# olegiy/manuscript-ocr

Hardware: AMD Instinct MI355X
Metric: manuscript pages/sec end-to-end (EAST+TRBA) at 1/2/4/8 MI355X; CER vs CPU ref (higher is better)
Workload: dtype f32 (bf16x3 split operands on the 1x1 / Winograd-domain GEMMs, f32 accumulate)

## Files before the change

### include/msocr.h

```cpp
#ifndef MSOCR_H
#define MSOCR_H
#include <stdint.h>

#ifdef __cplusplus
extern "C" {
#endif

#define MSOCR_F32 0
#define MSOCR_BF16 1

#define MSOCR_OK 0
#define MSOCR_E_ARG (-1)
#define MSOCR_E_LAUNCH (-2)
#define MSOCR_E_NOGPU (-3)

#define MSOCR_CONV_RELU 1u
#define MSOCR_CONV_RESIDUAL 2u
#define MSOCR_CONV_POOL2 4u

typedef struct msocr_conv_desc {
  int32_t dtype;
  int32_t N, H, W, Cin;
  int64_t in_sN, in_sH, in_sW;
  int32_t KH, KW, stride_h, stride_w, pad_h, pad_w;
  int32_t Ho, Wo, Cout;
  int64_t out_ld;
  int64_t res_ld;
  uint32_t flags;
} msocr_conv_desc;

int msocr_conv2d(const msocr_conv_desc* d, const void* in, const void* weight, const float* bias,
                 const void* residual, void* out, void* stream);

#define MSOCR_WINO_2X2 0
#define MSOCR_WINO_4X2 1
#define MSOCR_WINO_4X4 2
#define MSOCR_WINO_4X4_COLTAIL 3
int64_t msocr_winograd_workspace_bytes(const msocr_conv_desc* d, int form);
int msocr_winograd_weights_host(int form, const float* w_khwc_host, int Cout, int Cin, float* u_out_host);
int msocr_conv3x3_winograd(const msocr_conv_desc* d, int form, int split, const void* in, const void* u, const float* bias,
                           const void* residual, void* out, void* workspace, void* stream);
int msocr_winograd_input_transform(const msocr_conv_desc* d, int form, const void* in, void* workspace, void* stream);
int msocr_winograd_gemm(const msocr_conv_desc* d, int form, int split, const void* u, void* workspace, void* stream);
int msocr_winograd_output_transform(const msocr_conv_desc* d, int form, const void* workspace, const float* bias, const void* residual,
                                    void* out, void* stream);

int64_t msocr_winograd_crop_lds_bytes(const msocr_conv_desc* d, int form, int se);
int msocr_winograd_output_chain(const msocr_conv_desc* d, int form, void* workspace, const float* bias, void* stream);
int msocr_winograd_output_se(const msocr_conv_desc* d, int form, const void* workspace, const float* bias, const void* identity,
                             const float* w1, const float* w2, float* gate_ws, void* out, void* stream);

int msocr_split_bf16x3_host(const float* w_host, int64_t n, uint16_t* planes_out_host);
int msocr_split_bf16x3_ktile_host(const float* w_host, int64_t nbatch, int64_t rows, int64_t k, uint16_t* planes_out_host);
int msocr_conv1x1_split(const msocr_conv_desc* d, const void* in, const void* weight_planes, const float* bias,
                        const void* residual, void* out, void* stream);
int msocr_conv2d_split(const msocr_conv_desc* d, const void* in, const void* weight_planes, const float* bias,
                       const void* residual, void* out, void* stream);

int64_t msocr_winograd_fused64_workspace_bytes(const msocr_conv_desc* d);
int msocr_conv3x3_winograd_fused64(const msocr_conv_desc* d, int split, const void* in, const void* u, const float* bias,
                                   const void* residual, void* out, void* workspace, void* stream);
int msocr_winograd_fused64_gemm_output(const msocr_conv_desc* d, int split, const void* u, const void* workspace, const float* bias,
                                       const void* residual, void* out, void* stream);

int msocr_normalize_u8(const uint8_t* src, int N, int H, int W, int pad_t, int pad_l, int Hp, int Wp, int cpad,
                       int mode, int dtype, void* out, void* stream);

int msocr_resize_linear_u8(const uint8_t* src, int N, int sh, int sw, uint8_t* dst, int dh, int dw, void* stream);

int msocr_maxpool2d(const void* in, int N, int H, int W, int C, int64_t in_ld, int k, int s, int p, int dtype,
                    void* out, int Ho, int Wo, int64_t out_ld, void* stream);

int msocr_upsample2x_bilinear(const void* in, int N, int H, int W, int C, int64_t in_ld, int dtype, void* out,
                              int64_t out_ld, void* stream);

int msocr_east_head(const void* h1, int64_t npix, int64_t in_ld, int dtype, const float* w9, const float* b9,
                    float* score_out, float* geo_out, void* stream);

int msocr_east_decode(const float* score, const float* geo, int N, int H, int W, float thresh, float scale,
                      int quant, float* cand_out, int32_t* count_out, int max_cand, void* stream);

int64_t msocr_lanms_workspace_bytes(int N, int max_cand);
int msocr_east_lanms(const float* cand, const int32_t* counts, int N, int max_cand, double iou_thr, float* boxes_out,
                     int32_t* nbox_out, void* workspace, void* stream);

int64_t msocr_east_box_tail_workspace_bytes(int N, int max_cand);
int msocr_east_box_tail(const float* boxes, const int32_t* nbox, int N, int max_cand, double expand_w, double expand_h,
                        double scale_x, double scale_y, int axis_aligned_output, int remove_anomalies, double sigma, int min_count,
                        float* out, int32_t* n_out, void* workspace, void* stream);
int msocr_east_box_tail_host(const float* quads_host, int M, double expand_w, double expand_h, double scale_x, double scale_y,
// ... 260 lines not shown
```

### manuscript_ocr_amd/_native.py

```python
import ctypes
import os

import torch

_HERE = os.path.dirname(os.path.abspath(__file__))
LIB_PATH = os.path.join(_HERE, "libmsocr.so")

F32, BF16 = 0, 1
CONV_RELU, CONV_RESIDUAL, CONV_POOL2 = 1, 2, 4
WINO_2X2, WINO_4X2, WINO_4X4, WINO_4X4_COLTAIL = 0, 1, 2, 3

c_i32, c_i64, c_u32 = ctypes.c_int32, ctypes.c_int64, ctypes.c_uint32
c_f32, c_f64, c_vp = ctypes.c_float, ctypes.c_double, ctypes.c_void_p


class ConvDesc(ctypes.Structure):
    _fields_ = [
        ("dtype", c_i32), ("N", c_i32), ("H", c_i32), ("W", c_i32), ("Cin", c_i32),
        ("in_sN", c_i64), ("in_sH", c_i64), ("in_sW", c_i64),
        ("KH", c_i32), ("KW", c_i32), ("stride_h", c_i32), ("stride_w", c_i32), ("pad_h", c_i32), ("pad_w", c_i32),
        ("Ho", c_i32), ("Wo", c_i32), ("Cout", c_i32),
        ("out_ld", c_i64), ("res_ld", c_i64), ("flags", c_u32),
    ]

# ... 26 lines not shown

ATTN_GREEDY, ATTN_BEAM, ATTN_FORCED = 0, 1, 2


class AttnDesc(ctypes.Structure):
    _fields_ = (
        [(n, c_i32) for n in ("struct_bytes", "mode", "B", "T", "H", "V", "steps", "beam", "sos_id", "eos_id", "blank_id")]
        + [("temperature", c_f32), ("batch_H", c_vp), ("proj_H", c_vp), ("ctx_gates", c_vp),
           ("w", ctypes.POINTER(AttnWeights)), ("ws", ctypes.POINTER(AttnSplitWeights))]
        + [(n, c_vp) for n in ("lp", "tok_in", "logits_out", "ids_out", "workspace", "fin_step_out", "chunk_id", "chunk_size",
                               "chunk_state", "alpha_out")]
        + [("lexicon", ctypes.POINTER(LexiconArrays)), ("node_out", c_vp), ("lm", ctypes.POINTER(CharLMTable)), ("lm_weight", c_f32),
           ("ctx_out", c_vp)])


_SIGS = {
    "msocr_conv2d": (c_i32, [ctypes.POINTER(ConvDesc), c_vp, c_vp, c_vp, c_vp, c_vp, c_vp]),
    "msocr_winograd_workspace_bytes": (c_i64, [ctypes.POINTER(ConvDesc), c_i32]),
    "msocr_winograd_weights_host": (c_i32, [c_i32, c_vp, c_i32, c_i32, c_vp]),
    "msocr_conv3x3_winograd": (c_i32, [ctypes.POINTER(ConvDesc), c_i32, c_i32, c_vp, c_vp, c_vp, c_vp, c_vp, c_vp, c_vp]),
    "msocr_winograd_input_transform": (c_i32, [ctypes.POINTER(ConvDesc), c_i32, c_vp, c_vp, c_vp]),
    "msocr_winograd_gemm": (c_i32, [ctypes.POINTER(ConvDesc), c_i32, c_i32, c_vp, c_vp, c_vp]),
    "msocr_winograd_output_transform": (c_i32, [ctypes.POINTER(ConvDesc), c_i32, c_vp, c_vp, c_vp, c_vp, c_vp]),
    "msocr_winograd_crop_lds_bytes": (c_i64, [ctypes.POINTER(ConvDesc), c_i32, c_i32]),
    "msocr_winograd_output_chain": (c_i32, [ctypes.POINTER(ConvDesc), c_i32, c_vp, c_vp, c_vp]),
    "msocr_winograd_output_se": (c_i32, [ctypes.POINTER(ConvDesc), c_i32, c_vp, c_vp, c_vp, c_vp, c_vp, c_vp, c_vp, c_vp]),
    "msocr_winograd_fused64_workspace_bytes": (c_i64, [ctypes.POINTER(ConvDesc)]),
    "msocr_conv3x3_winograd_fused64": (c_i32, [ctypes.POINTER(ConvDesc), c_i32, c_vp, c_vp, c_vp, c_vp, c_vp, c_vp, c_vp]),
    "msocr_winograd_fused64_gemm_output": (c_i32, [ctypes.POINTER(ConvDesc), c_i32, c_vp, c_vp, c_vp, c_vp, c_vp, c_vp]),
    "msocr_split_bf16x3_host": (c_i32, [c_vp, c_i64, c_vp]),
    "msocr_split_bf16x3_ktile_host": (c_i32, [c_vp, c_i64, c_i64, c_i64, c_vp]),
    "msocr_conv1x1_split": (c_i32, [ctypes.POINTER(ConvDesc), c_vp, c_vp, c_vp, c_vp, c_vp, c_vp]),
    "msocr_conv2d_split": (c_i32, [ctypes.POINTER(ConvDesc), c_vp, c_vp, c_vp, c_vp, c_vp, c_vp]),
    "msocr_normalize_u8": (c_i32, [c_vp, c_i32, c_i32, c_i32, c_i32, c_i32, c_i32, c_i32, c_i32, c_i32, c_i32, c_vp, c_vp]),
    "msocr_resize_linear_u8": (c_i32, [c_vp, c_i32, c_i32, c_i32, c_vp, c_i32, c_i32, c_vp]),
    "msocr_maxpool2d": (c_i32, [c_vp, c_i32, c_i32, c_i32, c_i32, c_i64, c_i32, c_i32, c_i32, c_i32, c_vp, c_i32, c_i32, c_i64, c_vp]),
    "msocr_upsample2x_bilinear": (c_i32, [c_vp, c_i32, c_i32, c_i32, c_i32, c_i64, c_i32, c_vp, c_i64, c_vp]),
    "msocr_east_head": (c_i32, [c_vp, c_i64, c_i64, c_i32, c_vp, c_vp, c_vp, c_vp, c_vp]),
    "msocr_east_decode": (c_i32, [c_vp, c_vp, c_i32, c_i32, c_i32, c_f32, c_f32, c_i32, c_vp, c_vp, c_i32, c_vp]),
    "msocr_lanms_workspace_bytes": (c_i64, [c_i32, c_i32]),
    "msocr_east_lanms": (c_i32, [c_vp, c_vp, c_i32, c_i32, c_f64, c_vp, c_vp, c_vp, c_vp]),
    "msocr_se_residual": (c_i32, [c_vp, c_vp, c_i32, c_i32, c_i32, c_i32, c_vp, c_vp, c_vp, c_vp, c_vp]),
    "msocr_mean_over_h": (c_i32, [c_vp, c_i32, c_i32, c_i32, c_i32, c_i32, c_vp, c_vp]),
    "msocr_bilstm_recurrent": (c_i32, [c_vp, c_vp, c_i32, c_i32, c_i32, c_vp, c_vp]),
    "msocr_bilstm_recurrent_split": (c_i32, [c_vp, c_vp, c_i32, c_i32, c_i32, c_vp, c_vp]),
    "msocr_attn_pack_split_elems": (c_i64, [c_i32]),
    "msocr_attn_pack_split_host": (c_i32, [c_vp, c_i32, c_i32, c_vp]),
    "msocr_attn_beam_workspace_bytes": (c_i64, [c_i32, c_i32, c_i32, c_i32]),
    "msocr_attn_beam_finalize": (c_i32, [c_vp, c_i32, c_i32, c_i32, c_i32, c_vp, c_vp, c_vp, c_vp, c_i32, c_vp, c_vp]),
    "msocr_attn_beam_slots_bytes": (c_i64, [c_i32, c_i32, c_i32]),
    "msocr_attn_decode": (c_i32, [ctypes.POINTER(AttnDesc), c_vp]),
    "msocr_seq_confidence": (c_i32, [c_vp, c_vp, c_vp, c_i32, c_i32, c_i32, c_vp, c_vp]),
    "msocr_attn_beam_alpha_bytes": (c_i64, [c_i32, c_i32, c_i32, c_i32]),
    "msocr_seq_char_details": (c_i32, [c_vp, c_vp, c_vp, c_vp, c_i32, c_i32, c_i32, c_i32, c_vp, c_vp, c_vp, c_vp]),
    "msocr_attn_beam_nbest": (c_i32, [c_vp, c_i32, c_i32, c_i32, c_i32, c_i32, c_i32, c_vp, c_vp, c_vp, c_vp, c_vp, c_vp]),
    "msocr_attn_beam_nbest_host": (c_i32, [c_vp, c_i32, c_i32, c_i32, c_i32, c_i32, c_i32, c_vp, c_vp, c_vp, c_vp, c_vp]),
    "msocr_seq_logp": (c_i32, [c_vp, c_vp, c_vp, c_i32, c_i32, c_i32, c_f32, c_vp, c_vp, c_vp]),
    "msocr_seq_logp_host": (c_i32, [c_vp, c_vp, c_vp, c_i32, c_i32, c_i32, c_f32, c_vp, c_vp]),
    "msocr_lexicon_check_host": (c_i32, [c_vp, c_vp, c_vp, c_vp, c_i32, c_i32, c_i32, c_i32]),
    "msocr_lexicon_nearest_ws_bytes": (c_i64, [c_i32, c_i32, c_i32]),
    "msocr_lexicon_nearest": (c_i32, [c_vp, c_vp, c_i32, c_i32, c_i32, c_i32, c_i32, c_i32, ctypes.POINTER(WordList), c_i32, c_i32,
                                      c_vp, c_vp, c_vp, c_vp]),
    "msocr_lexicon_nearest_host": (c_i32, [c_vp, c_vp, c_i32, c_i32, c_i32, c_i32, c_i32, c_i32, ctypes.POINTER(WordList), c_i32, c_i32,
                                           c_vp, c_vp]),
    "msocr_edit_distance_pairs": (c_i32, [c_vp, c_vp, c_i32, c_vp, c_vp, c_i32, c_i32, c_i32, c_i32, c_i32, c_i32, c_vp, c_vp, c_vp,
                                          c_vp]),
# ... 105 lines not shown
```

### manuscript_ocr_amd/csrc/conv_common.h

```cpp
#ifndef MSOCR_CONV_COMMON_H
#define MSOCR_CONV_COMMON_H
#include <hip/hip_runtime.h>
#include <stdint.h>

#include <type_traits>

#include "internal.h"
#include "msocr.h"
#include "split_mma.h"

typedef uint32_t u32x4 __attribute__((ext_vector_type(4)));
typedef uint32_t u32x2 __attribute__((ext_vector_type(2)));

struct ConvParams {
  const char* in;
  const char* w;
  const float* bias;
  const char* res;
  char* out;
  int N, H, W, Cin;
  long sN, sH, sW;
  int KH, KW, SH, SW, PH, PW;
  int Ho, Wo, Cout;
  long M;
  int ktiles, cin_tiles;
  long Ktot;
  long out_ld, res_ld;
  int relu, has_res;
  int tilesM, tilesN;
  int nbatch;
  long bsA, bsW, bsO;
  long wplane;
  long w_kt_b;
};

__device__ __forceinline__ float bf16_to_f32(uint16_t v) { return __uint_as_float(((uint32_t)v) << 16); }
__device__ __forceinline__ uint16_t f32_to_bf16(float f) {
  __bf16 b = (__bf16)f;
  return *reinterpret_cast<uint16_t*>(&b);
}

template <typename T>
struct Mma;
template <>
struct Mma<float> {
  static __device__ __forceinline__ void run(const u32x4& a, const u32x4& b, f32x16& c) {
#pragma unroll
    for (int j = 0; j < 4; ++j)
      c = __builtin_amdgcn_mfma_f32_32x32x2f32(__uint_as_float(a[j]), __uint_as_float(b[j]), c, 0, 0, 0);
  }
};
template <>
struct Mma<__bf16> {
  static __device__ __forceinline__ void run(const u32x4& a, const u32x4& b, f32x16& c) {
    bf16x8 av = __builtin_bit_cast(bf16x8, a);
    bf16x8 bv = __builtin_bit_cast(bf16x8, b);
    c = __builtin_amdgcn_mfma_f32_32x32x16_bf16(av, bv, c, 0, 0, 0);
  }
};

__attribute__((visibility("hidden"))) bool msocr_internal_split_pp_takes(const ConvParams& p);
__attribute__((visibility("hidden"))) int msocr_internal_split_pp_launch(ConvParams& p, hipStream_t s, bool general);

template <int BKB>
__device__ __forceinline__ int swz(int row) {
  constexpr int CPR = BKB / 16;
// ... 2 lines not shown
}
__device__ __forceinline__ int swz16(int row) { return (4 - ((row >> 2) & 3)) & 3; }
template <typename T, int BM_, int BN_, int BKB_, int WM_, int STAGES_>
struct IgemmTile {
  static constexpr int BM = BM_, BN = BN_, BKB = BKB_, THREADS = 256, PERSISTENT = 0;
  static constexpr int BK = BKB / (int)sizeof(T);
  static constexpr int CPR = BKB / 16;
  static constexpr int RPP = 256 / CPR;
  static constexpr int A_IT = BM / RPP, B_IT = (BN + RPP - 1) / RPP;
  static constexpr int A_BYTES = BM * BKB, B_BYTES = BN * BKB, STAGE = A_BYTES + B_BYTES;
  static constexpr int EPI = (BM / WM_) * 32 * BN * 4;
  static constexpr int LDS = STAGES_ * STAGE > EPI ? STAGES_ * STAGE : EPI;
};
template <int BM_, int BN_>
struct SplitStage {
  static constexpr int BM = BM_, BN = BN_, BK = 32;
  static constexpr int ROWB = BK * 2;
  static constexpr int A_PLANE = BM * ROWB, B_PLANE = BN * ROWB;
  static constexpr int STAGE_B = 3 * (A_PLANE + B_PLANE);
  static constexpr int ACH = BK / 4, ARP = 256 / ACH, A_IT = BM / ARP;
  static constexpr int BCH = BK / 8, BRP = 256 / BCH, B_IT = (BN + BRP - 1) / BRP;
};
template <int BN_>
struct SplitTile : SplitStage<128, BN_> {
  static constexpr int WM = 64, WN = BN_ / 2, THREADS = 256, PERSISTENT = 0;
  static constexpr int EPI = (128 / WM) * 32 * BN_ * 4;
  static constexpr int LDS = SplitStage<128, BN_>::STAGE_B > EPI ? SplitStage<128, BN_>::STAGE_B : EPI;
  static __device__ __forceinline__ int swz(int row) { return ::swz<64>(row); }
};
template <int TM, int TN>
struct SplitPPTile : SplitStage<64 * TM, 64 * TN> {
  static constexpr int THREADS = 512, PERSISTENT = 1;
  static constexpr int BIAS_OFF = 2 * SplitStage<64 * TM, 64 * TN>::STAGE_B;
  static constexpr int LDS = BIAS_OFF + 4 * 64 * TN * 4;
  static __device__ __forceinline__ int swz(int row) { return swz16(row); }
};

static __device__ __attribute__((aligned(16))) uint32_t msocr_zero16[4] = {0u, 0u, 0u, 0u};

template <typename I>
__device__ __forceinline__ void xcd_range(I x, I nblk, I& first, I& count) {
  const I q = nblk >> 3, r = nblk & 7;
  first = x < r ? x * (q + 1) : r * (q + 1) + (x - r) * q;
  count = q + (x < r ? 1 : 0);
}
template <typename I>
__device__ __forceinline__ I xcd_tile(I bid, I nblk) {
  I first, count;
  xcd_range<I>(bid & 7, nblk, first, count);
  return first + (bid >> 3);
}
__device__ __forceinline__ void tile_coords(const ConvParams& p, int t, int& batch, int& tile_m, int& tile_n) {
  const int nblk1 = p.tilesM * p.tilesN;
  batch = t / nblk1;
  t -= batch * nblk1;
  tile_n = t % p.tilesN;
  tile_m = t / p.tilesN;
}

template <bool GEN>
struct ATap { int hi0, wi0; };
template <>
struct ATap<false> {};
__device__ __forceinline__ long a_row_origin(const ConvParams& p, long m, ATap<true>& t) {
  const long hw = (long)p.Ho * p.Wo;
  const int n = (int)(m / hw);
  const int rem = (int)(m - (long)n * hw);
// ... 42 lines not shown
}
__device__ __forceinline__ uint32_t b_plane_offset(int co, int cout, int b_chunk) {
  if (co >= cout) co = cout - 1;
  return (uint32_t)(co * 64 + b_chunk * 16);
}
template <class G>
__device__ __forceinline__ void load_b_planes(const ConvParams& p, const char* g_w, long wplane_b, int kt, int b_row0,
                                              const uint32_t (&b_off)[G::B_IT], u32x4 (&rb)[3][G::B_IT]) {
#pragma unroll
  for (int pl = 0; pl < 3; ++pl) {
    const char* const gb = g_w + pl * wplane_b + (long)kt * p.w_kt_b;
#pragma unroll
    for (int j = 0; j < G::B_IT; ++j)
      if (G::BN % G::BRP == 0 || b_row0 + j * G::BRP < G::BN) rb[pl][j] = *reinterpret_cast<const u32x4*>(gb + b_off[j]);
  }
}
template <class G>
__device__ __forceinline__ void split_store_row(unsigned char* sA, int row, int a_chunk, u32x4 r) {
  float x0 = __uint_as_float(r[0]), x1 = __uint_as_float(r[1]), x2 = __uint_as_float(r[2]), x3 = __uint_as_float(r[3]);
  unsigned char* dst = sA + row * G::ROWB + (((a_chunk >> 1) ^ G::swz(row)) << 4) + ((a_chunk & 1) << 3);
#pragma unroll
  for (int pl = 0; pl < 3; ++pl) {
    u32x2 v;
    v[0] = split_step(x0, x1);
    v[1] = split_step(x2, x3);
    *reinterpret_cast<u32x2*>(dst + pl * G::A_PLANE) = v;
  }
}
template <class G>
__device__ __forceinline__ void store_b_row(unsigned char* sB, int pl, int row, int b_chunk, u32x4 v) {
  *reinterpret_cast<u32x4*>(sB + pl * G::B_PLANE + row * G::ROWB + ((b_chunk ^ G::swz(row)) << 4)) = v;
}

template <typename T, int BM, int BN, int WM, int WN, int MT, bool BIAS16, int NCH = 1, typename AccT, int TMA, int TN>
__device__ __forceinline__ void epilogue_lds(const ConvParams& p, unsigned char* smem, const AccT (&acc)[TMA][TN], int tile_m, int tile_n,
                                             char* g_out, int wm, int wn, int r32, int half) {
  constexpr int ES = sizeof(T), EPC = 16 / ES;
  constexpr int AE = MT == 32 ? 16 : 4;
  const int tid = threadIdx.x;
  constexpr int PR = (BM / WM) * 32;
  float* sc = reinterpret_cast<float*>(smem);
  constexpr int VPR = BN / EPC;
  constexpr int ROWS_PP = 256 / VPR;
  const int vcol = (tid % VPR) * EPC;
  const int vrow0 = tid / VPR;
  const int co = tile_n * BN + vcol;
  float bias[EPC];
  if constexpr (BIAS16) {
    static_assert(EPC == 4, "four f32");
    f32x4 b = {0.f, 0.f, 0.f, 0.f};
    if (p.bias) b = *reinterpret_cast<const f32x4*>(p.bias + co);
    bias[0] = b[0]; bias[1] = b[1]; bias[2] = b[2]; bias[3] = b[3];
  } else {
#pragma unroll
    for (int e = 0; e < EPC; ++e) bias[e] = p.bias ? p.bias[co + e] : 0.f;
  }

  constexpr int TPP = 32 / MT;
  constexpr int NR = PR / ROWS_PP;
  static_assert(PR % ROWS_PP == 0 && NR % NCH == 0, "a pass is whole sweeps of 256 threads, a chunk whole rows");
  static_assert(32 % ROWS_PP == 0 || ROWS_PP == 64, "tile_row must be additive in the sweep index (see row_step)");
  const long m0 = (long)tile_m * BM;
  auto tile_row = [&](int i, int lr) { return (lr >> 5) * WM + i * 32 + (lr & 31); };
  auto lds_write = [&](int i) {
#pragma unroll
    for (int ti = 0; ti < TPP; ++ti)
// ... 147 lines not shown
  p.nbatch = 1;
  return p;
}
static inline int gemm_params(const void* A, const void* B, void* C, long M, int N, int K, int nbatch, int n_mult, int k_mult, ConvParams* out) {
  if (!A || !B || !C || M <= 0 || N <= 0 || N % n_mult || K <= 0 || K % k_mult || nbatch <= 0) return MSOCR_E_ARG;
  if (((uintptr_t)A | (uintptr_t)B | (uintptr_t)C) & 15) return MSOCR_E_ARG;
  if (M > 0x7fffffffL) return MSOCR_E_ARG;
  ConvParams p = {};
  p.in = (const char*)A; p.w = (const char*)B; p.out = (char*)C;
  p.N = 1; p.H = (int)M; p.W = 1; p.Cin = K;
  p.sN = M * (long)K; p.sH = K; p.sW = K;
  p.KH = p.KW = 1; p.SH = p.SW = 1;
  p.Ho = (int)M; p.Wo = 1; p.Cout = N;
  p.M = M; p.Ktot = K;
  p.out_ld = N;
  p.nbatch = nbatch; p.bsA = M * (long)K; p.bsW = (long)N * K; p.bsO = M * (long)N;
  *out = p;
  return MSOCR_OK;
}
template <class G, class Kern>
static int conv_launch(Kern kern, ConvParams& p, hipStream_t s) {
  p.tilesM = (int)((p.M + G::BM - 1) / G::BM);
  p.tilesN = p.Cout / G::BN;
  p.cin_tiles = p.Cin / G::BK;
  p.ktiles = (int)(p.Ktot / G::BK);
  if (msocr_internal_lds_limit(reinterpret_cast<const void*>(kern), G::LDS) != MSOCR_OK) return MSOCR_E_LAUNCH;
  const long nblk = (long)p.tilesM * p.tilesN * p.nbatch;
  if (nblk <= 0 || nblk > 0x7fffffffL) return MSOCR_E_ARG;
  long grid = nblk;
  if (G::PERSISTENT) {
    int n_cu = 0;
    if (msocr_internal_cu_count(&n_cu) != MSOCR_OK) return MSOCR_E_LAUNCH;
    n_cu = n_cu > 8 ? n_cu & ~7 : 8;
    grid = (nblk + 7) & ~7L;
    if (grid > n_cu) grid = n_cu;
  }
  MSOCR_LAUNCH(kern, dim3((unsigned)grid), dim3(G::THREADS), G::LDS, s, p);
  return hipGetLastError() == hipSuccess ? MSOCR_OK : MSOCR_E_LAUNCH;
}

#endif
```

### manuscript_ocr_amd/csrc/conv_split.hip

```cpp
#include <hip/hip_runtime.h>
#include <stdint.h>
#include <stdlib.h>
#include <string.h>

#include "conv_common.h"

namespace {

template <int BN, int WPE, bool GEN>
__global__ __launch_bounds__(256, WPE) void conv_split_kernel(ConvParams p) {
  using G = SplitTile<BN>;
  constexpr int BM = G::BM, WM = G::WM, WN = G::WN, BK = G::BK;
  constexpr int TM = WM / 32, TN = WN / 32;
  constexpr int ROWB = G::ROWB, A_PLANE = G::A_PLANE, B_PLANE = G::B_PLANE, STAGE_B = G::STAGE_B;
  constexpr int ACH = G::ACH, ARP = G::ARP, A_IT = G::A_IT;
  constexpr int BCH = G::BCH, B_IT = G::B_IT;

  extern __shared__ __attribute__((aligned(16))) unsigned char smem[];

  const int tid = threadIdx.x;
  const int lane = tid & 63;
  const int wave = tid >> 6;
  const int wm = wave >> 1, wn = wave & 1;

// ... 172 lines not shown
  return launch_split_any(p, (hipStream_t)stream, false);
}

extern "C" int msocr_conv2d_split(const msocr_conv_desc* d, const void* in, const void* weight_planes, const float* bias,
                                  const void* residual, void* out, void* stream) {
  if (!d || d->dtype != MSOCR_F32) return MSOCR_E_ARG;
  if (conv_desc_check(d, in, weight_planes, residual, out, 4, 32, 64, CONV_STRIDES_ALIGNED) != MSOCR_OK) return MSOCR_E_ARG;
  ConvParams p = conv_params(d, in, weight_planes, bias, residual, out);
  p.wplane = (long)d->Cout * p.Ktot;
  const long img_bytes = (long)d->in_sN * 4;
  if (img_bytes >= (1L << 31)) return MSOCR_E_ARG;
  const int per = (int)(((1L << 31) - 1) / (img_bytes > 0 ? img_bytes : 1));
  if (d->N <= per) return launch_split_any(p, (hipStream_t)stream, true);
  const long out_img = (long)d->Ho * d->Wo * d->out_ld * 4, res_img = (long)d->Ho * d->Wo * d->res_ld * 4;
  for (int n0 = 0; n0 < d->N; n0 += per) {
    ConvParams q = p;
    q.N = d->N - n0 < per ? d->N - n0 : per;
    q.M = (long)q.N * d->Ho * d->Wo;
    q.in = p.in + (long)n0 * img_bytes;
    q.out = p.out + (long)n0 * out_img;
    if (p.has_res) q.res = p.res + (long)n0 * res_img;
    const int rc = launch_split_any(q, (hipStream_t)stream, true);
    if (rc != MSOCR_OK) return rc;
  }
  return MSOCR_OK;
}

int msocr_internal_gemm_split_batched(const float* A, const uint16_t* Bplanes, float* C, long M, int N, int K, int nbatch, hipStream_t s) {
  ConvParams p;
  if (gemm_params(A, Bplanes, C, M, N, K, nbatch, 64, 32, &p) != MSOCR_OK) return MSOCR_E_ARG;
  p.wplane = (long)nbatch * N * K;
  return launch_split_any(p, s, false);
}
```

### manuscript_ocr_amd/csrc/conv_split_pp.hip

```cpp
#include <hip/hip_runtime.h>
#include <stdint.h>

#include <type_traits>

#include "conv_common.h"

namespace {

template <int I>
using ic = std::integral_constant<int, I>;
template <int U, int N, class F>
__device__ __forceinline__ void static_for(F&& f) {
  if constexpr (U < N) {
    f(ic<U>{});
    static_for<U + 1, N>(f);
  }
}

__device__ __forceinline__ void lds_barrier() {
  __builtin_amdgcn_sched_barrier(0);
  asm volatile("s_waitcnt lgkmcnt(0)\n\ts_barrier" ::: "memory");
  __builtin_amdgcn_sched_barrier(0);
}

template <int OFF>
__device__ __forceinline__ void store_f32x4_saddr(const char* sbase, uint32_t voff, f32x4 v) {
  asm volatile("global_store_dwordx4 %0, %1, %2 offset:%3" ::"v"(voff), "v"(v), "s"(sbase), "n"(OFF) : "memory");
}

template <int TM, int TN, bool GEN>
__global__ __launch_bounds__(512, 2) void conv_split_pp_kernel(ConvParams p) {
  using Tile = SplitPPTile<TM, TN>;
  constexpr int BM = Tile::BM, BN = Tile::BN, BK = Tile::BK, ROWB = Tile::ROWB;
  constexpr int A_PLANE = Tile::A_PLANE, B_PLANE = Tile::B_PLANE, STAGE_B = Tile::STAGE_B;
  constexpr int BIAS_OFF = Tile::BIAS_OFF;
  constexpr int RM = 2 * TM, RN = 2 * TN;
  constexpr bool STREAM_B = TN >= TM;
  constexpr int RH = STREAM_B ? RM : RN, RS = STREAM_B ? RN : RM;

  extern __shared__ __attribute__((aligned(16))) unsigned char smem[];

  const int tid = threadIdx.x;
  const int lane = tid & 63;
  const int wave = __builtin_amdgcn_readfirstlane(tid >> 6);

  const int nblk = p.tilesM * p.tilesN * p.nbatch;
  const int xcd = blockIdx.x & 7, slot = blockIdx.x >> 3, per_x = gridDim.x >> 3;
  int x_start, x_cnt;
  xcd_range<int>(xcd, nblk, x_start, x_cnt);
  const int my_tiles = slot < x_cnt ? (x_cnt - slot + per_x - 1) / per_x : 0;
  const int G = my_tiles * p.ktiles;
  if (G == 0) return;

  auto tile_of = [&](int n, int& batch, int& tile_m, int& tile_n) __attribute__((always_inline)) {
    tile_coords(p, x_start + slot + n * per_x, batch, tile_m, tile_n);
  };

  if (wave >= 4) {
    constexpr int D = 2;
    const int ltid = tid & 255;
    constexpr int ACH = Tile::ACH, ARP = Tile::ARP, A_IT = Tile::A_IT;
    constexpr int BCH = Tile::BCH, B_IT = Tile::B_IT;
    const int a_chunk = ltid % ACH, a_row0 = ltid / ACH;
    const int b_chunk = ltid % BCH, b_row0 = ltid / BCH;
    const long wplane_b = p.wplane * 2;
    const int bias_i = ltid < BN ? ltid : BN - 1;

    uint32_t a_off[A_IT], b_off[B_IT];
    ATap<GEN> a_tap[A_IT];
    const char* ga_base = nullptr;
    const char* gb_base = nullptr;
    const float* gbias = nullptr;
    int an = 0, akt = 0, bn = 0, bkt = 0;
    int sn = 0, skt = 0;
    TapCursor tap;
    tap.reset();

    auto set_tile_a = [&](int n) __attribute__((always_inline)) {
      int batch, tile_m, tile_n;
      tile_of(n, batch, tile_m, tile_n);
      ga_base = p.in + (long)batch * p.bsA * 4;
#pragma unroll
      for (int i = 0; i < A_IT; ++i) a_off[i] = a_row_offset32<GEN>(p, (long)tile_m * BM + a_row0 + i * ARP, a_chunk, a_tap[i]);
      tap.reset();
    };
    auto set_tile_b = [&](int n) __attribute__((always_inline)) {
      int batch, tile_m, tile_n;
      tile_of(n, batch, tile_m, tile_n);
      gb_base = p.w + (long)batch * p.bsW * 2;
      gbias = p.bias ? p.bias + tile_n * BN + bias_i : reinterpret_cast<const float*>(msocr_zero16);
#pragma unroll
      for (int j = 0; j < B_IT; ++j) b_off[j] = b_plane_offset(tile_n * BN + b_row0 + j * Tile::BRP, p.Cout, b_chunk);
    };

    u32x4 ra[D][A_IT], rb[D][3][B_IT];
    float rbias[D];
    auto load_a = [&](auto buf_c) __attribute__((always_inline)) {
      constexpr int BUF = decltype(buf_c)::value;
      if constexpr (GEN) load_a_taps32(p, ga_base, a_off, a_tap, tap, BK, ra[BUF]);
      else load_a_rows32(ga_base + (long)akt * (BK * 4), a_off, ra[BUF]);
      if (++akt == p.ktiles) {
        akt = 0;
        if (an + 1 < my_tiles) set_tile_a(++an);
        else tap.reset();
      }
    };
    auto load_b = [&](auto buf_c) __attribute__((always_inline)) {
      constexpr int BUF = decltype(buf_c)::value;
      rbias[BUF] = *gbias;
      load_b_planes<Tile>(p, gb_base, wplane_b, bkt, b_row0, b_off, rb[BUF]);
      if (++bkt == p.ktiles) {
        bkt = 0;
        if (bn + 1 < my_tiles) set_tile_b(++bn);
      }
    };
    auto store = [&](auto buf_c, int stage) __attribute__((always_inline)) {
      constexpr int BUF = decltype(buf_c)::value;
      unsigned char* const sA = smem + stage * STAGE_B;
#pragma unroll
      for (int i = 0; i < A_IT; ++i) split_store_row<Tile>(sA, a_row0 + i * ARP, a_chunk, ra[BUF][i]);
      unsigned char* const sB = sA + 3 * A_PLANE;
#pragma unroll
      for (int pl = 0; pl < 3; ++pl)
#pragma unroll
        for (int j = 0; j < B_IT; ++j) store_b_row<Tile>(sB, pl, b_row0 + j * Tile::BRP, b_chunk, rb[BUF][pl][j]);
      if (BN == 256 || ltid < BN) *reinterpret_cast<float*>(smem + BIAS_OFF + ((sn & 3) * BN + ltid) * 4) = rbias[BUF];
      if (++skt == p.ktiles) { skt = 0; ++sn; }
    };

    set_tile_a(0);
    set_tile_b(0);
    load_b(ic<0>{});
    load_a(ic<0>{});
    load_b(ic<1>{});
    load_a(ic<1>{});
    store(ic<0>{}, 0);
    lds_barrier();
    for (int g = 0;;) {
      load_b(ic<0>{});
      load_a(ic<0>{});
      store(ic<1>{}, 1);
      lds_barrier();
      if (++g >= G) break;
      load_b(ic<1>{});
      load_a(ic<1>{});
      store(ic<0>{}, 0);
      lds_barrier();
      if (++g >= G) break;
    }
    return;
  }

  __builtin_amdgcn_s_setprio(1);
  const int wm = wave >> 1, wn = wave & 1;
  const int r16 = lane & 15, kg = lane >> 4;
  const uint32_t c16 = (uint32_t)((kg ^ swz16(r16)) << 4);
  const uint32_t offA = (uint32_t)((wm * 32 * TM + r16) * ROWB) + c16;
  const uint32_t offB = (uint32_t)(3 * A_PLANE + (wn * 32 * TN + r16) * ROWB) + c16;
  const uint32_t offH = STREAM_B ? offA : offB, offS = STREAM_B ? offB : offA;
  constexpr int PLANE_H = STREAM_B ? A_PLANE : B_PLANE, PLANE_S = STREAM_B ? B_PLANE : A_PLANE;

  bf16x8 fh[3][RH], fs[2][3];
  auto read_held = [&](auto h_c, uint32_t so) __attribute__((always_inline)) {
    constexpr int H = decltype(h_c)::value;
#pragma unroll
    for (int pl = 0; pl < 3; ++pl) fh[pl][H] = *reinterpret_cast<const bf16x8*>(smem + so + offH + pl * PLANE_H + H * 16 * ROWB);
  };
  auto read_stream = [&](auto s_c, uint32_t so) __attribute__((always_inline)) {
    constexpr int S = decltype(s_c)::value;
#pragma unroll
    for (int pl = 0; pl < 3; ++pl) fs[S & 1][pl] = *reinterpret_cast<const bf16x8*>(smem + so + offS + pl * PLANE_S + S * 16 * ROWB);
  };

  f32x4 acc[RM][RN];
  f32x4 part[2][RH];
  auto chain = [&](auto s_c, auto h_c) __attribute__((always_inline)) {
    constexpr int S = decltype(s_c)::value, H = decltype(h_c)::value;
    f32x4 t = {0.f, 0.f, 0.f, 0.f};
#pragma unroll
    for (int k = 0; k < 6; ++k) {
      if constexpr (STREAM_B) t = __builtin_amdgcn_mfma_f32_16x16x32_bf16(fs[S & 1][split_pb(k)], fh[split_pa(k)][H], t, 0, 0, 0);
      else t = __builtin_amdgcn_mfma_f32_16x16x32_bf16(fh[split_pb(k)][H], fs[S & 1][split_pa(k)], t, 0, 0, 0);
    }
    part[S & 1][H] = t;
  };
  auto commit = [&](auto s_c, auto h_c, auto first_c) __attribute__((always_inline)) {
    constexpr int S = decltype(s_c)::value, H = decltype(h_c)::value;
    f32x4& a = STREAM_B ? acc[H][S] : acc[S][H];
    if constexpr (decltype(first_c)::value != 0) a = part[S & 1][H];
    else a += part[S & 1][H];
    asm volatile("" : "+v"(a));
  };

  char* e_ob = nullptr;
  int e_lim = 0;
  bool e_full = true;
  int e_slot = 0;
  const float lo = p.relu ? 0.f : -__builtin_inff();
  const uint32_t vo = (uint32_t)((r16 * p.out_ld + 4 * kg) * 4);
  auto set_epilogue = [&](int n) __attribute__((always_inline)) {
    int batch, tile_m, tile_n;
    tile_of(n, batch, tile_m, tile_n);
    const long row0 = (long)tile_m * BM + wm * 32 * TM;
    const int col0 = tile_n * BN + wn * 32 * TN;
    e_ob = p.out + ((long)batch * p.bsO + row0 * p.out_ld + col0) * 4;
    const long rows = p.M - row0;
    e_full = rows >= 32 * TM;
    e_lim = (int)(rows < 32 * TM ? rows : 32 * TM) - r16;
    e_slot = n & 3;
  };
  auto store_blocks = [&](auto s_c) __attribute__((always_inline)) {
    constexpr int S = decltype(s_c)::value;
    const long ld16 = p.out_ld * 64;
    const float* const sbias = reinterpret_cast<const float*>(smem + BIAS_OFF) + e_slot * BN + wn * 32 * TN + 4 * kg;
    auto body = [&](auto masked_c) __attribute__((always_inline)) {
      constexpr bool MASKED = decltype(masked_c)::value != 0;
      static_for<0, RH>([&](auto h_c) __attribute__((always_inline)) {
        constexpr int H = decltype(h_c)::value;
        constexpr int I = STREAM_B ? H : S, J = STREAM_B ? S : H;
        const f32x4 b4 = *reinterpret_cast<const f32x4*>(sbias + J * 16);
        f32x4 v = acc[I][J] + b4;
        v[0] = fmaxf(v[0], lo); v[1] = fmaxf(v[1], lo); v[2] = fmaxf(v[2], lo); v[3] = fmaxf(v[3], lo);
        const char* const rowp = e_ob + I * ld16;
        if (!MASKED || I * 16 < e_lim) store_f32x4_saddr<J * 64>(rowp, vo, v);
      });
    };
    if (e_full) body(ic<0>{});
    else body(ic<1>{});
  };

  uint32_t so = 0;
  auto ktile = [&](auto first_c, auto pend_first_c, bool prev) __attribute__((always_inline)) {
    constexpr int FIRST = decltype(first_c)::value;
    static_for<0, RS - 1>([&](auto u_c) __attribute__((always_inline)) {
      constexpr int U = decltype(u_c)::value;
      read_stream(ic<U + 1>{}, so);
      __builtin_amdgcn_sched_barrier(0);
      if constexpr (FIRST != 0) {
        if (prev) store_blocks(u_c);
        __builtin_amdgcn_sched_barrier(0);
      }
      static_for<0, RH>([&](auto h_c) __attribute__((always_inline)) {
        chain(u_c, h_c);
        if constexpr (U > 0) commit(ic<U - 1>{}, h_c, first_c);
        else if (FIRST == 0 || prev) commit(ic<RS - 1>{}, h_c, pend_first_c);
      });
      __builtin_amdgcn_sched_barrier(0);
    });
    lds_barrier();
    so ^= (uint32_t)STAGE_B;
    read_stream(ic<0>{}, so);
    __builtin_amdgcn_sched_barrier(0);
    if constexpr (FIRST != 0) {
      if (prev) store_blocks(ic<RS - 1>{});
      __builtin_amdgcn_sched_barrier(0);
    }
    static_for<0, RH>([&](auto h_c) __attribute__((always_inline)) {
      chain(ic<RS - 1>{}, h_c);
      commit(ic<RS - 2>{}, h_c, first_c);
      __builtin_amdgcn_sched_barrier(0);
      read_held(h_c, so);
      __builtin_amdgcn_sched_barrier(0);
    });
  };

  lds_barrier();
  static_for<0, RH>([&](auto h_c) __attribute__((always_inline)) { read_held(h_c, so); });
  read_stream(ic<0>{}, so);
  for (int n = 0; n < my_tiles; ++n) {
    ktile(ic<1>{}, ic<0>{}, n > 0);
    set_epilogue(n);
    ktile(ic<0>{}, ic<1>{}, false);
    for (int kt = 2; kt < p.ktiles; ++kt) ktile(ic<0>{}, ic<0>{}, false);
  }
  static_for<0, RH>([&](auto h_c) __attribute__((always_inline)) { commit(ic<RS - 1>{}, h_c, ic<0>{}); });
  static_for<0, RS>([&](auto s_c) __attribute__((always_inline)) { store_blocks(s_c); });
}

template <int TM, int TN, bool GEN>
int launch_pp(ConvParams& p, hipStream_t s) {
  return conv_launch<SplitPPTile<TM, TN>>(conv_split_pp_kernel<TM, TN, GEN>, p, s);
}

}

bool msocr_internal_split_pp_takes(const ConvParams& p) { return p.Cout % 128 == 0 && !p.has_res && p.Ktot >= 64; }

int msocr_internal_split_pp_launch(ConvParams& p, hipStream_t s, bool general) {
  if (p.Cout % 256 == 0) return general ? launch_pp<2, 4, true>(p, s) : launch_pp<2, 4, false>(p, s);
  if (p.Cout % 128 == 0) return general ? launch_pp<4, 2, true>(p, s) : launch_pp<4, 2, false>(p, s);
  return MSOCR_E_ARG;
}
```

Measured before the change: 83.98.

## Schedule persistent split GEMM tiles with per-XCD atomic ticket work stealing

Replaces the static round-robin tile assignment in the persistent split-bf16x3 conv/GEMM kernel with dynamic claiming through global atomic ticket counters, one per XCD. A block that finishes its own XCD range can steal tiles from other XCDs, which evens out load imbalance. Claimed tile ids go through a small LDS ring read by the loader and epilogue waves. It also adds a configurable CU reserve that shrinks the persistent grid, plus a batched GEMM entry point. The cost is atomic traffic, cross-XCD cache locality loss on stolen tiles, and per-stream ticket slot bookkeeping on the host, which takes a mutex on every launch.

```diff
diff --git a/include/msocr.h b/include/msocr.h
--- a/include/msocr.h
+++ b/include/msocr.h
@@ -56,6 +56,11 @@
                         const void* residual, void* out, void* stream);
 int msocr_conv2d_split(const msocr_conv_desc* d, const void* in, const void* weight_planes, const float* bias,
                        const void* residual, void* out, void* stream);
+
+int msocr_gemm_split_batched(const float* A, const uint16_t* b_planes, float* C, int64_t M, int N, int K, int nbatch, void* stream);
+
+int msocr_set_gemm_cu_reserve(int reserve);
+int msocr_get_gemm_cu_reserve(void);
 
 int64_t msocr_winograd_fused64_workspace_bytes(const msocr_conv_desc* d);
 int msocr_conv3x3_winograd_fused64(const msocr_conv_desc* d, int split, const void* in, const void* u, const float* bias,
diff --git a/manuscript_ocr_amd/_native.py b/manuscript_ocr_amd/_native.py
--- a/manuscript_ocr_amd/_native.py
+++ b/manuscript_ocr_amd/_native.py
@@ -82,6 +82,9 @@
     "msocr_split_bf16x3_ktile_host": (c_i32, [c_vp, c_i64, c_i64, c_i64, c_vp]),
     "msocr_conv1x1_split": (c_i32, [ctypes.POINTER(ConvDesc), c_vp, c_vp, c_vp, c_vp, c_vp, c_vp]),
     "msocr_conv2d_split": (c_i32, [ctypes.POINTER(ConvDesc), c_vp, c_vp, c_vp, c_vp, c_vp, c_vp]),
+    "msocr_gemm_split_batched": (c_i32, [c_vp, c_vp, c_vp, c_i64, c_i32, c_i32, c_i32, c_vp]),
+    "msocr_set_gemm_cu_reserve": (c_i32, [c_i32]),
+    "msocr_get_gemm_cu_reserve": (c_i32, []),
     "msocr_normalize_u8": (c_i32, [c_vp, c_i32, c_i32, c_i32, c_i32, c_i32, c_i32, c_i32, c_i32, c_i32, c_i32, c_vp, c_vp]),
     "msocr_resize_linear_u8": (c_i32, [c_vp, c_i32, c_i32, c_i32, c_vp, c_i32, c_i32, c_vp]),
     "msocr_maxpool2d": (c_i32, [c_vp, c_i32, c_i32, c_i32, c_i32, c_i64, c_i32, c_i32, c_i32, c_i32, c_vp, c_i32, c_i32, c_i64, c_vp]),
diff --git a/manuscript_ocr_amd/csrc/conv_common.h b/manuscript_ocr_amd/csrc/conv_common.h
--- a/manuscript_ocr_amd/csrc/conv_common.h
+++ b/manuscript_ocr_amd/csrc/conv_common.h
@@ -32,6 +32,7 @@
   long bsA, bsW, bsO;
   long wplane;
   long w_kt_b;
+  int ticket_slot;
 };
 
 __device__ __forceinline__ float bf16_to_f32(uint16_t v) { return __uint_as_float(((uint32_t)v) << 16); }
@@ -100,7 +101,8 @@
 struct SplitPPTile : SplitStage<64 * TM, 64 * TN> {
   static constexpr int THREADS = 512, PERSISTENT = 1;
   static constexpr int BIAS_OFF = 2 * SplitStage<64 * TM, 64 * TN>::STAGE_B;
-  static constexpr int LDS = BIAS_OFF + 4 * 64 * TN * 4;
+  static constexpr int RING_OFF = BIAS_OFF + 4 * 64 * TN * 4;
+  static constexpr int LDS = RING_OFF + 16;
   static __device__ __forceinline__ int swz(int row) { return swz16(row); }
 };
 
@@ -422,6 +424,8 @@
     int n_cu = 0;
     if (msocr_internal_cu_count(&n_cu) != MSOCR_OK) return MSOCR_E_LAUNCH;
     n_cu = n_cu > 8 ? n_cu & ~7 : 8;
+    const int reserve = msocr_get_gemm_cu_reserve();
+    n_cu = n_cu - reserve > 8 ? n_cu - reserve : 8;
     grid = (nblk + 7) & ~7L;
     if (grid > n_cu) grid = n_cu;
   }
diff --git a/manuscript_ocr_amd/csrc/conv_split.hip b/manuscript_ocr_amd/csrc/conv_split.hip
--- a/manuscript_ocr_amd/csrc/conv_split.hip
+++ b/manuscript_ocr_amd/csrc/conv_split.hip
@@ -228,3 +228,6 @@
   p.wplane = (long)nbatch * N * K;
   return launch_split_any(p, s, false);
 }
+extern "C" int msocr_gemm_split_batched(const float* A, const uint16_t* b_planes, float* C, int64_t M, int N, int K, int nbatch, void* stream) {
+  return msocr_internal_gemm_split_batched(A, b_planes, C, (long)M, N, K, nbatch, (hipStream_t)stream);
+}
diff --git a/manuscript_ocr_amd/csrc/conv_split_pp.hip b/manuscript_ocr_amd/csrc/conv_split_pp.hip
--- a/manuscript_ocr_amd/csrc/conv_split_pp.hip
+++ b/manuscript_ocr_amd/csrc/conv_split_pp.hip
@@ -1,6 +1,10 @@
 #include <hip/hip_runtime.h>
 #include <stdint.h>
 
+#include <atomic>
+#include <map>
+#include <mutex>
+#include <tuple>
 #include <type_traits>
 
 #include "conv_common.h"
@@ -28,12 +32,44 @@
   asm volatile("global_store_dwordx4 %0, %1, %2 offset:%3" ::"v"(voff), "v"(v), "s"(sbase), "n"(OFF) : "memory");
 }
 
+constexpr int PP_SLOTS = 4096, PP_SLOT_WORDS = 16, PP_LEFT = 8;
+__device__ uint32_t msocr_pp_tickets[PP_SLOTS * PP_SLOT_WORDS];
+
+__device__ __forceinline__ uint32_t ticket_add(uint32_t* w) { return __hip_atomic_fetch_add(w, 1u, __ATOMIC_RELAXED, __HIP_MEMORY_SCOPE_AGENT); }
+__device__ __forceinline__ void pp_leave(uint32_t* tk) {
+  if (ticket_add(tk + PP_LEFT) != gridDim.x - 1) return;
+  for (int i = 0; i <= PP_LEFT; ++i) __hip_atomic_store(tk + i, 0u, __ATOMIC_RELAXED, __HIP_MEMORY_SCOPE_AGENT);
+}
+__device__ __forceinline__ int pp_claim(uint32_t* tk, int nblk, int xcd, int per_x, int lane) {
+  auto range = [&](int l, int& first, int& count, int& by_position) __attribute__((always_inline)) {
+    xcd_range<int>((xcd + l) & 7, nblk, first, count);
+    by_position = count < per_x ? count : per_x;
+  };
+  for (;;) {
+    int first, count, by_position;
+    range(lane & 7, first, count, by_position);
+    const uint32_t seen = __hip_atomic_load(tk + ((xcd + lane) & 7), __ATOMIC_RELAXED, __HIP_MEMORY_SCOPE_AGENT);
+    const unsigned long long open = __ballot(lane < 8 && (uint32_t)by_position + seen < (uint32_t)count);
+    if (!open) {
+      if (lane == 0) pp_leave(tk);
+      return -1;
+    }
+    const int l = __builtin_ctzll(open);
+    range(l, first, count, by_position);
+    uint32_t t = 0;
+    if (lane == 0) t = (uint32_t)by_position + ticket_add(tk + ((xcd + l) & 7));
+    t = (uint32_t)__builtin_amdgcn_readfirstlane((int)t);
+    if (t < (uint32_t)count) return first + (int)t;
+  }
+}
+
 template <int TM, int TN, bool GEN>
 __global__ __launch_bounds__(512, 2) void conv_split_pp_kernel(ConvParams p) {
   using Tile = SplitPPTile<TM, TN>;
   constexpr int BM = Tile::BM, BN = Tile::BN, BK = Tile::BK, ROWB = Tile::ROWB;
   constexpr int A_PLANE = Tile::A_PLANE, B_PLANE = Tile::B_PLANE, STAGE_B = Tile::STAGE_B;
   constexpr int BIAS_OFF = Tile::BIAS_OFF;
+  constexpr int RING_OFF = Tile::RING_OFF;
   constexpr int RM = 2 * TM, RN = 2 * TN;
   constexpr bool STREAM_B = TN >= TM;
   constexpr int RH = STREAM_B ? RM : RN, RS = STREAM_B ? RN : RM;
@@ -48,13 +84,13 @@
   const int xcd = blockIdx.x & 7, slot = blockIdx.x >> 3, per_x = gridDim.x >> 3;
   int x_start, x_cnt;
   xcd_range<int>(xcd, nblk, x_start, x_cnt);
-  const int my_tiles = slot < x_cnt ? (x_cnt - slot + per_x - 1) / per_x : 0;
-  const int G = my_tiles * p.ktiles;
-  if (G == 0) return;
-
-  auto tile_of = [&](int n, int& batch, int& tile_m, int& tile_n) __attribute__((always_inline)) {
-    tile_coords(p, x_start + slot + n * per_x, batch, tile_m, tile_n);
-  };
+  uint32_t* const tk = msocr_pp_tickets + p.ticket_slot * PP_SLOT_WORDS;
+  if (slot >= x_cnt) {
+    if (tid == 0) pp_leave(tk);
+    return;
+  }
+  int* const ring = reinterpret_cast<int*>(smem + RING_OFF);
+  auto ring_at = [&](int n) __attribute__((always_inline)) { return __builtin_amdgcn_readfirstlane(ring[n & 3]); };
 
   if (wave >= 4) {
     constexpr int D = 2;
@@ -72,21 +108,22 @@
     const char* gb_base = nullptr;
     const float* gbias = nullptr;
     int an = 0, akt = 0, bn = 0, bkt = 0;
+    int G = p.ktiles;
     int sn = 0, skt = 0;
     TapCursor tap;
     tap.reset();
 
-    auto set_tile_a = [&](int n) __attribute__((always_inline)) {
+    auto set_tile_a = [&](int t) __attribute__((always_inline)) {
       int batch, tile_m, tile_n;
-      tile_of(n, batch, tile_m, tile_n);
+      tile_coords(p, t, batch, tile_m, tile_n);
       ga_base = p.in + (long)batch * p.bsA * 4;
 #pragma unroll
       for (int i = 0; i < A_IT; ++i) a_off[i] = a_row_offset32<GEN>(p, (long)tile_m * BM + a_row0 + i * ARP, a_chunk, a_tap[i]);
       tap.reset();
     };
-    auto set_tile_b = [&](int n) __attribute__((always_inline)) {
+    auto set_tile_b = [&](int t) __attribute__((always_inline)) {
       int batch, tile_m, tile_n;
-      tile_of(n, batch, tile_m, tile_n);
+      tile_coords(p, t, batch, tile_m, tile_n);
       gb_base = p.w + (long)batch * p.bsW * 2;
       gbias = p.bias ? p.bias + tile_n * BN + bias_i : reinterpret_cast<const float*>(msocr_zero16);
 #pragma unroll
@@ -97,22 +134,34 @@
     float rbias[D];
     auto load_a = [&](auto buf_c) __attribute__((always_inline)) {
       constexpr int BUF = decltype(buf_c)::value;
+      if (akt == p.ktiles) {
+        akt = 0;
+        const int t = ring_at(an + 1);
+        if (t >= 0) { ++an; set_tile_a(t); }
+        else tap.reset();
+      }
       if constexpr (GEN) load_a_taps32(p, ga_base, a_off, a_tap, tap, BK, ra[BUF]);
       else load_a_rows32(ga_base + (long)akt * (BK * 4), a_off, ra[BUF]);
-      if (++akt == p.ktiles) {
-        akt = 0;
-        if (an + 1 < my_tiles) set_tile_a(++an);
-        else tap.reset();
-      }
+      ++akt;
     };
     auto load_b = [&](auto buf_c) __attribute__((always_inline)) {
       constexpr int BUF = decltype(buf_c)::value;
+      if (bkt == p.ktiles) {
+        bkt = 0;
+        const int t = ring_at(bn + 1);
+        if (t >= 0) {
+          ++bn;
+          G += p.ktiles;
+          set_tile_b(t);
+          if (wave == 4) {
+            const int next = pp_claim(tk, nblk, xcd, per_x, lane);
+            if (lane == 0) ring[(bn + 1) & 3] = next;
+          }
+        }
+      }
       rbias[BUF] = *gbias;
       load_b_planes<Tile>(p, gb_base, wplane_b, bkt, b_row0, b_off, rb[BUF]);
-      if (++bkt == p.ktiles) {
-        bkt = 0;
-        if (bn + 1 < my_tiles) set_tile_b(++bn);
-      }
+      ++bkt;
     };
     auto store = [&](auto buf_c, int stage) __attribute__((always_inline)) {
       constexpr int BUF = decltype(buf_c)::value;
@@ -128,12 +177,19 @@
       if (++skt == p.ktiles) { skt = 0; ++sn; }
     };
 
-    set_tile_a(0);
-    set_tile_b(0);
+    set_tile_a(x_start + slot);
+    set_tile_b(x_start + slot);
     load_b(ic<0>{});
     load_a(ic<0>{});
     load_b(ic<1>{});
     load_a(ic<1>{});
+    if (wave == 4) {
+      const int next = pp_claim(tk, nblk, xcd, per_x, lane);
+      if (lane == 0) {
+        ring[0] = x_start + slot;
+        ring[1] = next;
+      }
+    }
     store(ic<0>{}, 0);
     lds_barrier();
     for (int g = 0;;) {
@@ -196,11 +252,13 @@
   int e_lim = 0;
   bool e_full = true;
   int e_slot = 0;
+  bool e_more = false;
   const float lo = p.relu ? 0.f : -__builtin_inff();
   const uint32_t vo = (uint32_t)((r16 * p.out_ld + 4 * kg) * 4);
   auto set_epilogue = [&](int n) __attribute__((always_inline)) {
     int batch, tile_m, tile_n;
-    tile_of(n, batch, tile_m, tile_n);
+    tile_coords(p, ring_at(n), batch, tile_m, tile_n);
+    e_more = ring_at(n + 1) >= 0;
     const long row0 = (long)tile_m * BM + wm * 32 * TM;
     const int col0 = tile_n * BN + wn * 32 * TN;
     e_ob = p.out + ((long)batch * p.bsO + row0 * p.out_ld + col0) * 4;
@@ -267,22 +325,52 @@
   lds_barrier();
   static_for<0, RH>([&](auto h_c) __attribute__((always_inline)) { read_held(h_c, so); });
   read_stream(ic<0>{}, so);
-  for (int n = 0; n < my_tiles; ++n) {
+  for (int n = 0;; ++n) {
     ktile(ic<1>{}, ic<0>{}, n > 0);
     set_epilogue(n);
     ktile(ic<0>{}, ic<1>{}, false);
     for (int kt = 2; kt < p.ktiles; ++kt) ktile(ic<0>{}, ic<0>{}, false);
+    if (!e_more) break;
   }
   static_for<0, RH>([&](auto h_c) __attribute__((always_inline)) { commit(ic<RS - 1>{}, h_c, ic<0>{}); });
   static_for<0, RS>([&](auto s_c) __attribute__((always_inline)) { store_blocks(s_c); });
 }
 
+int pp_ticket_slot(hipStream_t s, int* slot) {
+  static std::mutex mu;
+  static std::map<std::tuple<unsigned long long, hipStream_t, int>, int> slots;
+  static std::atomic<int> threads{0};
+  thread_local const int thread_tag = ++threads;
+  hipStreamCaptureStatus st = hipStreamCaptureStatusNone;
+  unsigned long long capture = 0;
+  if (hipStreamGetCaptureInfo(s, &st, &capture) != hipSuccess) return MSOCR_E_LAUNCH;
+  if (st != hipStreamCaptureStatusActive) capture = 0;
+  const auto key = std::make_tuple(capture, s, s == hipStreamPerThread ? thread_tag : 0);
+  std::lock_guard<std::mutex> lock(mu);
+  auto it = slots.find(key);
+  if (it == slots.end()) {
+    if ((int)slots.size() >= PP_SLOTS) return MSOCR_E_LAUNCH;
+    it = slots.emplace(key, (int)slots.size()).first;
+  }
+  *slot = it->second;
+  return MSOCR_OK;
+}
+
 template <int TM, int TN, bool GEN>
 int launch_pp(ConvParams& p, hipStream_t s) {
+  if (pp_ticket_slot(s, &p.ticket_slot) != MSOCR_OK) return MSOCR_E_LAUNCH;
   return conv_launch<SplitPPTile<TM, TN>>(conv_split_pp_kernel<TM, TN, GEN>, p, s);
 }
 
 }
+
+static std::atomic<int> g_cu_reserve{0};
+extern "C" int msocr_set_gemm_cu_reserve(int reserve) {
+  if (reserve < 0 || reserve % 8) return MSOCR_E_ARG;
+  g_cu_reserve.store(reserve, std::memory_order_relaxed);
+  return MSOCR_OK;
+}
+extern "C" int msocr_get_gemm_cu_reserve(void) { return g_cu_reserve.load(std::memory_order_relaxed); }
 
 bool msocr_internal_split_pp_takes(const ConvParams& p) { return p.Cout % 128 == 0 && !p.has_res && p.Ktot >= 64; }
 
```

Result: slower. 83.01 (-1.2%).

## Stream B weight planes straight to LDS with global_load_lds DMA in producer waves

Applied to the files above, without the earlier changes.

The producer waves now copy the three bf16 weight planes for each k-tile directly from global memory into LDS using global_load_lds_dwordx4, instead of loading them into VGPRs and storing them to LDS. Each producer wave handles a quarter of the rows, and a vmcnt wait before the barrier ensures the DMA has landed. This removes register pressure and LDS store instructions on the B path, but it changes the prefetch depth for B from two register buffers to a direct stage write. It also relies on the swizzled lane layout and the vmcnt counting (A_IT younger loads) being correct. The bias load is also collapsed to a single register.

```diff
diff --git a/manuscript_ocr_amd/csrc/conv_common.h b/manuscript_ocr_amd/csrc/conv_common.h
--- a/manuscript_ocr_amd/csrc/conv_common.h
+++ b/manuscript_ocr_amd/csrc/conv_common.h
@@ -209,6 +209,40 @@
   *reinterpret_cast<u32x4*>(sB + pl * G::B_PLANE + row * G::ROWB + ((b_chunk ^ G::swz(row)) << 4)) = v;
 }
 
+template <class G>
+__device__ __forceinline__ uint32_t b_piece_lane_offset(int lane) {
+  static_assert(G::ROWB == 64 && G::BN % 64 == 0, "a piece is 16 whole rows; four producer waves share a plane evenly");
+  const int row = lane >> 2;
+  return (uint32_t)(row * G::ROWB + (((lane & 3) ^ G::swz(row)) << 4));
+}
+template <int OFF>
+__device__ __forceinline__ void lds_dma_piece(const char* sbase, uint32_t voff, uint32_t lds_dst) {
+  uint32_t keep;
+  asm volatile("s_mov_b32 %0, m0\n\ts_mov_b32 m0, %3\n\ts_nop 0\n\tglobal_load_lds_dwordx4 %1, %2 offset:%4\n\ts_mov_b32 m0, %0"
+               : "=&s"(keep)
+               : "v"(voff), "s"(sbase), "s"(lds_dst), "n"(OFF)
+               : "memory");
+}
+template <int YOUNGER>
+__device__ __forceinline__ void lds_dma_wait() {
+  asm volatile("s_waitcnt vmcnt(%0)" ::"n"(YOUNGER) : "memory");
+}
+template <class G>
+__device__ __forceinline__ void dma_b_planes(const char* gb, long wplane_b, uint32_t voff, uint32_t lds_b) {
+  static_assert(G::BN == 128 || G::BN == 256, "two or four pieces per plane and wave");
+#pragma unroll
+  for (int pl = 0; pl < 3; ++pl) {
+    const char* const g = gb + pl * wplane_b;
+    const uint32_t l = lds_b + pl * G::B_PLANE;
+    lds_dma_piece<0>(g, voff, l);
+    lds_dma_piece<1024>(g, voff, l);
+    if constexpr (G::BN == 256) {
+      lds_dma_piece<2048>(g, voff, l);
+      lds_dma_piece<3072>(g, voff, l);
+    }
+  }
+}
+
 template <typename T, int BM, int BN, int WM, int WN, int MT, bool BIAS16, int NCH = 1, typename AccT, int TMA, int TN>
 __device__ __forceinline__ void epilogue_lds(const ConvParams& p, unsigned char* smem, const AccT (&acc)[TMA][TN], int tile_m, int tile_n,
                                              char* g_out, int wm, int wn, int r32, int half) {
diff --git a/manuscript_ocr_amd/csrc/conv_split_pp.hip b/manuscript_ocr_amd/csrc/conv_split_pp.hip
--- a/manuscript_ocr_amd/csrc/conv_split_pp.hip
+++ b/manuscript_ocr_amd/csrc/conv_split_pp.hip
@@ -59,14 +59,15 @@
   if (wave >= 4) {
     constexpr int D = 2;
     const int ltid = tid & 255;
+    const int pw = wave - 4;
     constexpr int ACH = Tile::ACH, ARP = Tile::ARP, A_IT = Tile::A_IT;
-    constexpr int BCH = Tile::BCH, B_IT = Tile::B_IT;
     const int a_chunk = ltid % ACH, a_row0 = ltid / ACH;
-    const int b_chunk = ltid % BCH, b_row0 = ltid / BCH;
     const long wplane_b = p.wplane * 2;
     const int bias_i = ltid < BN ? ltid : BN - 1;
-
-    uint32_t a_off[A_IT], b_off[B_IT];
+    const uint32_t b_voff = b_piece_lane_offset<Tile>(lane);
+    const uint32_t b_lds = (uint32_t)(uintptr_t)(__attribute__((address_space(3))) unsigned char*)smem + 3 * A_PLANE + pw * (BN / 4) * ROWB;
+
+    uint32_t a_off[A_IT];
     ATap<GEN> a_tap[A_IT];
     const char* ga_base = nullptr;
     const char* gb_base = nullptr;
@@ -87,14 +88,12 @@
     auto set_tile_b = [&](int n) __attribute__((always_inline)) {
       int batch, tile_m, tile_n;
       tile_of(n, batch, tile_m, tile_n);
-      gb_base = p.w + (long)batch * p.bsW * 2;
+      gb_base = p.w + (long)batch * p.bsW * 2 + (long)(tile_n * BN + pw * (BN / 4)) * ROWB;
       gbias = p.bias ? p.bias + tile_n * BN + bias_i : reinterpret_cast<const float*>(msocr_zero16);
-#pragma unroll
-      for (int j = 0; j < B_IT; ++j) b_off[j] = b_plane_offset(tile_n * BN + b_row0 + j * Tile::BRP, p.Cout, b_chunk);
-    };
-
-    u32x4 ra[D][A_IT], rb[D][3][B_IT];
-    float rbias[D];
+    };
+
+    u32x4 ra[D][A_IT];
+    float rbias;
     auto load_a = [&](auto buf_c) __attribute__((always_inline)) {
       constexpr int BUF = decltype(buf_c)::value;
       if constexpr (GEN) load_a_taps32(p, ga_base, a_off, a_tap, tap, BK, ra[BUF]);
@@ -105,10 +104,9 @@
         else tap.reset();
       }
     };
-    auto load_b = [&](auto buf_c) __attribute__((always_inline)) {
-      constexpr int BUF = decltype(buf_c)::value;
-      rbias[BUF] = *gbias;
-      load_b_planes<Tile>(p, gb_base, wplane_b, bkt, b_row0, b_off, rb[BUF]);
+    auto stage_b = [&](int stage) __attribute__((always_inline)) {
+      dma_b_planes<Tile>(gb_base + (long)bkt * p.w_kt_b, wplane_b, b_voff, b_lds + stage * STAGE_B);
+      rbias = *gbias;
       if (++bkt == p.ktiles) {
         bkt = 0;
         if (bn + 1 < my_tiles) set_tile_b(++bn);
@@ -119,33 +117,31 @@
       unsigned char* const sA = smem + stage * STAGE_B;
 #pragma unroll
       for (int i = 0; i < A_IT; ++i) split_store_row<Tile>(sA, a_row0 + i * ARP, a_chunk, ra[BUF][i]);
-      unsigned char* const sB = sA + 3 * A_PLANE;
-#pragma unroll
-      for (int pl = 0; pl < 3; ++pl)
-#pragma unroll
-        for (int j = 0; j < B_IT; ++j) store_b_row<Tile>(sB, pl, b_row0 + j * Tile::BRP, b_chunk, rb[BUF][pl][j]);
-      if (BN == 256 || ltid < BN) *reinterpret_cast<float*>(smem + BIAS_OFF + ((sn & 3) * BN + ltid) * 4) = rbias[BUF];
+      if (BN == 256 || ltid < BN) *reinterpret_cast<float*>(smem + BIAS_OFF + ((sn & 3) * BN + ltid) * 4) = rbias;
       if (++skt == p.ktiles) { skt = 0; ++sn; }
+    };
+    auto hand_over = [&]() __attribute__((always_inline)) {
+      lds_dma_wait<A_IT>();
+      lds_barrier();
     };
 
     set_tile_a(0);
     set_tile_b(0);
-    load_b(ic<0>{});
+    stage_b(0);
     load_a(ic<0>{});
-    load_b(ic<1>{});
     load_a(ic<1>{});
     store(ic<0>{}, 0);
-    lds_barrier();
+    hand_over();
     for (int g = 0;;) {
-      load_b(ic<0>{});
+      stage_b(1);
       load_a(ic<0>{});
       store(ic<1>{}, 1);
-      lds_barrier();
+      hand_over();
       if (++g >= G) break;
-      load_b(ic<1>{});
+      stage_b(0);
       load_a(ic<1>{});
       store(ic<0>{}, 0);
-      lds_barrier();
+      hand_over();
       if (++g >= G) break;
     }
     return;
```

Result: no change. 84.61 before, 85.69 after (median of 6 runs) (+1.3%).
